# jeongminpark417/COALA-GNN

Hardware: AMD Instinct MI355X
Metric: feature-gather GB/s (payload = rows x dim x 4 B delivered per second), IGB-medium GraphSAGE minibatch fetch (higher is better)
Workload: dtype f32

## Files before the change

coala-gnn_amd/csrc/coala_cache.hip:

```cpp
#include <hip/hip_runtime.h>
#include <hip/hip_ext.h>

#include <algorithm>
#include <cstdarg>
#include <cstdio>
#include <cstdlib>
#include <cstring>
#include <new>
#include <type_traits>
#include <utility>
#include <vector>

#include "../../include/coala_hip.h"
#include "coala_internal.h"

namespace {

constexpr uint64_t kEmptyKey = 0xFFFFFFFFFFFFFFFFull;
constexpr uint32_t kLinkMiss = 0x80000000u;
constexpr uint32_t kLinkBad = 0x7FFFFFFFu;
constexpr int kStatBlocks = 2048;
constexpr int kFillSlots = 8;

struct CacheDev {
    void* keys;
    uint64_t* set_cnt;
    uint32_t* color_meta;
    int32_t* color_counters;
    const int32_t* node_color;
    float* lines;
    const float* cold;
    uint64_t num_sets;
    uint64_t num_rows;
    uint32_t cache_dim;
    uint32_t dim;
    uint32_t n_gpus;
    int32_t gshift;
    int32_t sshift;
    uint32_t distributed;
    uint32_t cold_partitioned;
    uint32_t tag32;
    uint64_t* set_head;
    uint32_t* miss_link;
    unsigned long long* stats;
};

__device__ __forceinline__ uint64_t set_of(const CacheDev& c, uint64_t id) {
    uint64_t k = id;
    if (c.distributed) {
        if (c.gshift >= 0) k = id >> c.gshift;
        else if ((id >> 32) == 0) k = (uint32_t)id / c.n_gpus;
        else k = id / c.n_gpus;
    }
    if (c.sshift >= 0) return k & (c.num_sets - 1);
    if ((k >> 32) == 0 && (c.num_sets >> 32) == 0) return (uint32_t)k % (uint32_t)c.num_sets;
    return k % c.num_sets;
}

__device__ __forceinline__ uint64_t cold_row_of(const CacheDev& c, uint64_t id) {
    if (!c.cold_partitioned) return id;
    if (c.gshift >= 0) return id >> c.gshift;
    return id / c.n_gpus;
}

constexpr int kMaxRanges = 64;
struct RangeSet {
    uint32_t n;
// ... 52 lines not shown
template <int CD, int VEC, int NP = 4>
struct Geo {
    static constexpr int UNITS = CD / VEC;
    static constexpr int LPR = UNITS >= 64 ? 64 : UNITS;
    static constexpr int RPP = 64 / LPR;
    static constexpr int VPL = UNITS / LPR;
    static constexpr int PASSES = (VPL >= 16) ? 1 : NP;
    static constexpr int R = RPP * PASSES;
};

constexpr int kK1MinWaves = 4;
constexpr int kK1Passes = 4;
constexpr int64_t kK1SingleMaxChunks = 1 << 20;
constexpr int kK1Waves = 2;
#ifdef COALA_DEV_KNOBS
constexpr int kK1MaxWaves = 4;
#else
constexpr int kK1MaxWaves = kK1Waves;
#endif

template <typename V> __device__ __forceinline__ V nt_load(const V* p) { return __builtin_nontemporal_load(p); }
template <typename V> __device__ __forceinline__ void nt_store(V v, V* p) { __builtin_nontemporal_store(v, p); }

template <int CD, int VEC, typename TAG, int NP, bool FULL, bool REDIR, bool SINGLE>
__global__ __launch_bounds__(64 * kK1MaxWaves, kK1MinWaves) void probe_gather_kernel(const int64_t* __restrict__ idx, float* __restrict__ out,
                                                                    int64_t n, uint32_t gen, uint32_t n_blocks, CacheDev c, Redirect rd) {
    using G = Geo<CD, VEC, NP>;
    using V = typename VecT<VEC>::type;
    using TG = TagGeo<TAG>;
    using TV = typename TG::vec;
    constexpr int R = G::R;
    static_assert(R <= 32, "per-chunk row masks are 32 bits wide");
    if (blockIdx.x == 0 && threadIdx.x < kFillSlots) reinterpret_cast<uint32_t*>(c.stats + 2 * kStatBlocks)[(gen & 1u) * kFillSlots + threadIdx.x] = 0u;
    uint32_t* fill_flag = reinterpret_cast<uint32_t*>(c.stats + 2 * kStatBlocks) + 2 * kFillSlots;
    if (blockIdx.x == 0 && threadIdx.x == kFillSlots) fill_flag[(gen + 1u) & 1u] = 0u;
    constexpr int TSTEPS = (R + TG::SPL - 1) / TG::SPL;
    int lane = threadIdx.x & 63;
#ifdef COALA_DEV_KNOBS
    const int wpb = (int)(blockDim.x >> 6);
#else
    constexpr int wpb = kK1Waves;
#endif
    const int64_t wave = (int64_t)blockIdx.x * wpb + (threadIdx.x >> 6);
    const int64_t n_waves = (int64_t)n_blocks * wpb;
    const int64_t n_chunks = (n + R - 1) / R;
    const uint32_t nunits = c.dim / VEC;
    const TAG* __restrict__ keys = reinterpret_cast<const TAG*>(c.keys);

    struct Ids { uint64_t id[TSTEPS]; bool valid[TSTEPS]; int32_t drow[REDIR ? TSTEPS : 1]; };
    struct Tags { uint64_t id[TSTEPS]; uint32_t set[TSTEPS]; TV kk[TSTEPS]; bool ok[TSTEPS]; bool valid[TSTEPS]; int32_t drow[REDIR ? TSTEPS : 1]; };
    auto load_ids = [&](int64_t chunk) {
        Ids r;
#pragma unroll
        for (int t = 0; t < TSTEPS; ++t) {
            const int q_l = t * TG::SPL + lane / TG::LPS;
// ... 15 lines not shown
            r.id[t] = ids.id[t];
            r.valid[t] = ids.valid[t];
            if (REDIR) r.drow[t] = ids.drow[t];
            r.ok[t] = ids.valid[t] && ids.id[t] < c.num_rows;
            r.set[t] = r.ok[t] ? (uint32_t)set_of(c, ids.id[t]) : 0u;
            r.kk[t] = TV(TG::EMPTY);
            if (r.ok[t]) r.kk[t] = *reinterpret_cast<const TV*>(keys + (uint64_t)r.set[t] * COALA_WAYS + (lane % TG::LPS) * TG::KPL);
        }
        return r;
    };

    int64_t chunk = wave;
    Ids ids_next = load_ids(chunk);
    Tags tags = load_tags(ids_next);
    if (!SINGLE) ids_next = load_ids(chunk + n_waves);

    for (; chunk < n_chunks; chunk += n_waves) {
        asm volatile("" : "+v"(lane));
        const int64_t base = chunk * R;
        uint32_t slot_v[TSTEPS];
        int32_t drow_v[REDIR ? TSTEPS : 1];
        uint64_t hit_b[TSTEPS], bad_b[TSTEPS];
        bool lead_l[TSTEPS], imiss_l[TSTEPS], bad_l[TSTEPS];
        unsigned long long prev[TSTEPS];
        const uint32_t lane_way0 = (uint32_t)((lane % TG::LPS) * TG::KPL);
#pragma unroll
        for (int t = 0; t < TSTEPS; ++t) {
            const TAG want = (TAG)tags.id[t];
            uint32_t way = 0xFFu;
#pragma unroll
            for (int k = TG::KPL - 1; k >= 0; --k)
                if (tags.kk[t][k] == want) way = lane_way0 + (uint32_t)k;
            if (!tags.ok[t]) way = 0xFFu;
            way = umin_u32(way, dpp_u32<0xB1>(way));
            way = umin_u32(way, dpp_u32<0x4E>(way));
            way = umin_u32(way, dpp_u32<0x141>(way));
            if (TG::LPS == 16) way = umin_u32(way, dpp_u32<0x140>(way));
            const bool hit = way != 0xFFu;
            slot_v[t] = tags.set[t] * COALA_WAYS + (way & (COALA_WAYS - 1));
            if (REDIR) drow_v[t] = tags.drow[t];
            hit_b[t] = __ballot(hit);
            bad_l[t] = tags.valid[t] && !tags.ok[t];
            bad_b[t] = __ballot(bad_l[t]);
            lead_l[t] = tags.valid[t] && (lane % TG::LPS) == 0;
            imiss_l[t] = lead_l[t] && tags.ok[t] && !hit;
            prev[t] = 0;
            if (imiss_l[t]) {
                const unsigned long long tag = ((unsigned long long)gen << 32) | (unsigned long long)(base + t * TG::SPL + lane / TG::LPS + 1);
                prev[t] = atomicExch(reinterpret_cast<unsigned long long*>(c.set_head + tags.set[t]), tag);
            }
        }
        {
            bool any = false;
#pragma unroll
            for (int t = 0; t < TSTEPS; ++t) any = any || imiss_l[t] || bad_l[t];
            if (__ballot(any) != 0 && lane == 0) fill_flag[gen & 1u] = 1u;
        }
        auto row_slot = [&](int q) { return (uint32_t)__builtin_amdgcn_readlane((int)slot_v[q / TG::SPL], TG::LPS * (q % TG::SPL)); };
        auto row_hit = [&](int q) { return ((hit_b[q / TG::SPL] >> (TG::LPS * (q % TG::SPL))) & 1) != 0; };
        auto row_bad = [&](int q) { return ((bad_b[q / TG::SPL] >> (TG::LPS * (q % TG::SPL))) & 1) != 0; };
        Ids ids_next2;
        if (!SINGLE) ids_next2 = load_ids(chunk + 2 * n_waves);

        const int sub = (G::RPP == 2) ? (lane >> 5) : 0;
        const int l_in = lane & (G::LPR - 1);
        V val[G::PASSES][G::VPL];
#pragma unroll
        for (int p = 0; p < G::PASSES; ++p) {
            const uint32_t s_a = row_slot(p * G::RPP), s_b = row_slot(p * G::RPP + (G::RPP - 1));
            const bool h_a = row_hit(p * G::RPP), h_b = row_hit(p * G::RPP + (G::RPP - 1));
            const uint32_t s = (G::RPP == 2 && sub) ? s_b : s_a;
            const bool h = (G::RPP == 2 && sub) ? h_b : h_a;
            const V* src = reinterpret_cast<const V*>(c.lines + (uint64_t)s * CD);
#pragma unroll
            for (int v = 0; v < G::VPL; ++v) {
                const uint32_t u = v * G::LPR + l_in;
                if (h && (FULL || u < nunits)) val[p][v] = nt_load(src + u);
            }
        }
        if (!SINGLE) {
            tags = load_tags(ids_next);
            ids_next = ids_next2;
        }
#pragma unroll
        for (int p = 0; p < G::PASSES; ++p) {
            const int q = p * G::RPP + sub;
            const bool h_a = row_hit(p * G::RPP), h_b = row_hit(p * G::RPP + (G::RPP - 1));
            const bool bad_a = row_bad(p * G::RPP), bad_b2 = row_bad(p * G::RPP + (G::RPP - 1));
            const bool h = (G::RPP == 2 && sub) ? h_b : h_a;
            const bool bad = (G::RPP == 2 && sub) ? bad_b2 : bad_a;
            V* dst = reinterpret_cast<V*>(out + (base + q) * (int64_t)c.dim);
            if (REDIR) {
                auto row_drow = [&](int r) { return (int32_t)__builtin_amdgcn_readlane(drow_v[r / TG::SPL], TG::LPS * (r % TG::SPL)); };
                const int32_t dr_a = row_drow(p * G::RPP), dr_b = row_drow(p * G::RPP + (G::RPP - 1));
                const int32_t dr = (G::RPP == 2 && sub) ? dr_b : dr_a;
                if (dr >= 0) dst = reinterpret_cast<V*>(rd.out + (int64_t)dr * (int64_t)c.dim);
            }
#pragma unroll
            for (int v = 0; v < G::VPL; ++v) {
                const uint32_t u = v * G::LPR + l_in;
                if (FULL || u < nunits) {
                    if (h) dst[u] = val[p][v];
                    else if (bad) dst[u] = V(0.0f);
                }
            }
        }
#pragma unroll
        for (int t = 0; t < TSTEPS; ++t) {
            if (lead_l[t]) {
                uint32_t w = 0u;
                if (imiss_l[t]) w = kLinkMiss | (((uint32_t)(prev[t] >> 32) == gen) ? (uint32_t)prev[t] : 0u);
                else if (bad_l[t]) w = kLinkBad;
                c.miss_link[base + t * TG::SPL + lane / TG::LPS] = w;
            }
        }
        if (SINGLE) break;
    }
}

__device__ __forceinline__ uint64_t shfl64(uint64_t v, int src) {
    const uint32_t lo = __shfl((int)(uint32_t)v, src), hi = __shfl((int)(uint32_t)(v >> 32), src);
    return ((uint64_t)hi << 32) | lo;
}

template <int CD, int VEC, bool REDIR = false, int NP = 4>
__global__ __launch_bounds__(256) void miss_fill_kernel(CacheDev c, const int64_t* __restrict__ idx, float* __restrict__ out,
                                                        int tile_rows, int sparse_max, uint32_t gen, RangeSet rs, Redirect rd, int dyn_slot) {
    using G = Geo<CD, VEC, NP>;
    using V = typename VecT<VEC>::type;
    constexpr int R = G::R;
    const int lane = threadIdx.x & 63;
    const int64_t wave = (int64_t)blockIdx.x * (blockDim.x >> 6) + (threadIdx.x >> 6);
    const int64_t n_waves = (int64_t)gridDim.x * (blockDim.x >> 6);
    const int64_t n_tiles = ((int64_t)rs.total + tile_rows - 1) / tile_rows;
    const int chunks_per_tile = tile_rows / R;
    const uint32_t nunits = c.dim / VEC;
    const int sub = (G::RPP == 2) ? (lane >> 5) : 0;
    const int l_in = lane & (G::LPR - 1);
    uint32_t my_miss = 0, my_bad = 0;

    constexpr int U = 8;
    uint32_t* ticket = reinterpret_cast<uint32_t*>(c.stats + 2 * kStatBlocks) + (dyn_slot < 0 ? 0 : dyn_slot);
    const bool dyn = dyn_slot >= 0;
    if (reinterpret_cast<const uint32_t*>(c.stats + 2 * kStatBlocks)[2 * kFillSlots + (gen & 1u)] == 0u) return;
    const int64_t n_deal = dyn ? 1 : n_waves;
    const int64_t even8 = n_tiles / (n_waves * 8);
    const int claim_min = even8 < 1 ? 1 : (even8 > U ? U : (int)even8);
    int claim = claim_min;
    for (int64_t unit = dyn ? -1 : wave;;) {
      int64_t claim_end = n_tiles;
      if (dyn) {
          uint32_t t = 0;
          if (lane == 0) t = atomicAdd(ticket, (uint32_t)claim);
          unit = (int64_t)(uint32_t)__builtin_amdgcn_readfirstlane((int)t);
          if (unit >= n_tiles) break;
          claim_end = unit + claim < n_tiles ? unit + claim : n_tiles;
          claim = claim * 2 > 4 * U ? 4 * U : claim * 2;
      } else if (unit >= n_tiles) break;
     for (int64_t tile0 = unit; tile0 < claim_end; tile0 += n_deal * U) {
      const int n_here = dyn ? (int)(claim_end - tile0 < U ? claim_end - tile0 : U) : U;
      uint64_t st_pack = 0;
#pragma unroll
      for (int u = 0; u < U; ++u) {
          const int64_t tile = tile0 + u * n_deal;
          const uint32_t p = (u < n_here && tile < n_tiles && lane < tile_rows) ? pos_of(rs, (uint32_t)(tile * tile_rows + lane)) : 0xFFFFFFFFu;
          const uint32_t w = (p != 0xFFFFFFFFu) ? c.miss_link[p] : 0u;
          const uint64_t v = (w == 0u) ? 0u : ((w & kLinkMiss) ? 1u : 2u);
          st_pack |= v << (8 * u);
      }
      if (!__ballot(st_pack != 0)) continue;
      uint32_t slot_l = 0, win_l = 0;
      uint64_t id_l = 0;
      int64_t drow_l = 0;
      auto rank_at = [&](uint32_t pos) {
          id_l = (uint64_t)idx[pos];
          drow_l = (int64_t)pos;
          if (REDIR && (int64_t)pos >= rd.begin && (int64_t)pos < rd.end)
              drow_l = -((rd.row_map ? rd.row_map[(int64_t)pos - rd.begin] : (int64_t)pos - rd.begin) + 1);
          const uint64_t set = set_of(c, id_l);
          uint32_t cur = (uint32_t)c.set_head[set];
          uint32_t total = 0, rank = 0;
          while (cur) {
              const uint32_t p2 = cur - 1;
              ++total;
              rank += (p2 < pos) ? 1u : 0u;
              cur = c.miss_link[p2] & ~kLinkMiss;
          }
          const uint64_t cv = __hip_atomic_load(c.set_cnt + set, __ATOMIC_RELAXED, __HIP_MEMORY_SCOPE_AGENT);
          const uint32_t cnt0 = ((uint32_t)(cv >> 32) == gen) ? (uint32_t)cv - total : (uint32_t)cv;
          if (rank == 0) __hip_atomic_store(c.set_cnt + set, ((uint64_t)gen << 32) | (uint32_t)(cnt0 + total), __ATOMIC_RELAXED, __HIP_MEMORY_SCOPE_AGENT);
          const uint32_t way = (cnt0 + rank) & (COALA_WAYS - 1);
          slot_l = (uint32_t)(set * COALA_WAYS) + way;
          win_l = (rank + COALA_WAYS >= total) ? 1u : 0u;
          if (win_l) {
              if (c.tag32) reinterpret_cast<uint32_t*>(c.keys)[slot_l] = (uint32_t)id_l;
              else reinterpret_cast<uint64_t*>(c.keys)[slot_l] = id_l;
              if (c.color_counters) {
                  const int32_t col = c.node_color[id_l];
                  atomicSub(c.color_counters + c.color_meta[slot_l], 1);
                  atomicAdd(c.color_counters + col, 1);
                  c.color_meta[slot_l] = (uint32_t)col;
              }
          }
      };
      auto move_group = [&](const int (&srcl)[G::PASSES], const bool (&live)[G::PASSES]) {
          V val[G::PASSES][G::VPL];
          uint32_t slot_[G::PASSES];
          uint64_t id[G::PASSES];
          int64_t drow[G::PASSES];
          bool winner[G::PASSES];
#pragma unroll
          for (int p = 0; p < G::PASSES; ++p) {
              slot_[p] = (uint32_t)__shfl((int)slot_l, srcl[p]);
              winner[p] = __shfl((int)win_l, srcl[p]) != 0;
              id[p] = shfl64(id_l, srcl[p]);
              drow[p] = (int64_t)shfl64((uint64_t)drow_l, srcl[p]);
          }
#pragma unroll
          for (int p = 0; p < G::PASSES; ++p) {
              const V* src = reinterpret_cast<const V*>(c.cold + cold_row_of(c, id[p]) * (uint64_t)c.dim);
#pragma unroll
              for (int v = 0; v < G::VPL; ++v) {
                  const uint32_t u = v * G::LPR + l_in;
                  if (live[p] && u < nunits) val[p][v] = nt_load(src + u);
              }
// ... 40 lines not shown
          const uint32_t cnt = (uint32_t)__builtin_popcountll(mmask[u]);
          total_miss += cnt;
          worst = cnt > worst ? cnt : worst;
      }
      if (!total_miss) continue;
      claim = claim_min;
      if (total_miss <= 64 && (int)worst <= sparse_max) {
          uint32_t k = (uint32_t)lane;
          int u_sel = -1;
          uint64_t m_sel = 0;
#pragma unroll
          for (int u = 0; u < U; ++u) {
              const uint32_t cnt = (uint32_t)__builtin_popcountll(mmask[u]);
              if (u_sel < 0) {
                  if (k < cnt) { u_sel = u; m_sel = mmask[u]; }
                  else k -= cnt;
              }
          }
          if (u_sel >= 0) {
              for (uint32_t i = 0; i < k; ++i) m_sel &= m_sel - 1;
              const uint32_t pos = pos_of(rs, (uint32_t)((tile0 + u_sel * n_deal) * tile_rows + __builtin_ctzll(m_sel)));
              rank_at(pos);
          }
          stream_holders(total_miss >= 64 ? ~0ull : ((1ull << total_miss) - 1ull));
          continue;
      }
#pragma nounroll
      for (int u = 0; u < U; ++u) {
        const uint8_t st = (uint8_t)(st_pack >> (8 * u));
        const uint64_t tile_mask = __ballot(st == 1);
        if (!tile_mask) continue;
        const uint32_t pos_l = st ? pos_of(rs, (uint32_t)((tile0 + u * n_deal) * tile_rows + lane)) : 0u;
        if (__builtin_popcountll(tile_mask) <= sparse_max) {
            if (st == 1) rank_at(pos_l);
            stream_holders(tile_mask);
        } else {
            int srcl[G::PASSES];
            bool live[G::PASSES];
            for (int ck = 0; ck < chunks_per_tile; ++ck) {
                const uint32_t live_mask = (uint32_t)(tile_mask >> (ck * R)) & ((1u << R) - 1u);
                if (!live_mask) continue;
                const int lane0 = ck * R;
                if (st == 1 && lane >= lane0 && lane < lane0 + R) rank_at(pos_l);
#pragma unroll
                for (int p = 0; p < G::PASSES; ++p) {
                    const int q = p * G::RPP + sub;
                    live[p] = (live_mask >> q) & 1;
                    srcl[p] = lane0 + q;
                }
                move_group(srcl, live);
            }
        }
      }
     }
      if (!dyn) break;
    }
    __shared__ uint32_t s_m[256 / 64], s_b[256 / 64];
    for (int off = 32; off > 0; off >>= 1) { my_miss += __shfl_down(my_miss, off); my_bad += __shfl_down(my_bad, off); }
    if (lane == 0) { s_m[threadIdx.x >> 6] = my_miss; s_b[threadIdx.x >> 6] = my_bad; }
    __syncthreads();
    if (threadIdx.x == 0) {
        uint32_t m = 0, b = 0;
        for (int w = 0; w < (int)(blockDim.x >> 6); ++w) { m += s_m[w]; b += s_b[w]; }
        if (m) c.stats[2 * blockIdx.x] += m;
        if (b) c.stats[2 * blockIdx.x + 1] += b;
    }
// ... 124 lines not shown
            if ((uint32_t)lane == g) off += __builtin_popcountll(mask);
        }
        if (valid) {
            node_out[dest] = id;
            map_out[dest] = i;
        }
    }
}

}


namespace {

struct LaunchShape {
    int k1_grid_cap;
    int k1_waves;
    bool k1_single;
    int k1_passes;
    int k2_grid_cap;
    int k2_tile_rows;
    int k2_sparse_max;
    int k2_unit_tiles;
};

LaunchShape launch_shape(uint32_t cache_dim, bool host_tier) {
    LaunchShape s;
    s.k1_grid_cap = 16384;
    s.k1_waves = kK1Waves;
    s.k1_single = cache_dim >= 256;
    s.k1_passes = 0;
    const int host_blocks = std::min(64, std::max(24, 16 * 1024 / (int)cache_dim));
    s.k2_grid_cap = host_tier ? host_blocks : kStatBlocks;
    s.k2_tile_rows = host_tier ? 64 : 0;
    s.k2_sparse_max = host_tier ? 32 : 0;
    s.k2_unit_tiles = host_tier ? 1 : 0;
    return s;
}

#ifdef COALA_DEV_KNOBS
void apply_dev_knobs(LaunchShape& s) {
    if (const char* e = getenv("COALA_K1_PASSES")) { int v = atoi(e); if (v == 2 || v == 4 || v == 8 || v == 16) s.k1_passes = v; }
    if (const char* e = getenv("COALA_K1_GRID")) { int g = atoi(e); if (g >= 1 && g <= 65535) s.k1_grid_cap = g; }
    if (const char* e = getenv("COALA_K1_WAVES")) { int w = atoi(e); if (w == 1 || w == 2 || w == 4) s.k1_waves = w; }
    if (const char* e = getenv("COALA_K1_SINGLE")) s.k1_single = atoi(e) != 0;
    if (const char* e = getenv("COALA_K2_TILE_ROWS")) { int t = atoi(e); if (t == 0 || t == 8 || t == 16 || t == 32 || t == 64) s.k2_tile_rows = t; }
    if (const char* e = getenv("COALA_K2_GRID")) { int g = atoi(e); if (g >= 1 && g <= kStatBlocks) s.k2_grid_cap = g; }
    if (const char* e = getenv("COALA_K2_SPARSE")) { int g = atoi(e); if (g >= 0 && g <= 64) s.k2_sparse_max = g; }
    if (const char* e = getenv("COALA_K2_UNIT_TILES")) { int g = atoi(e); if (g >= 0 && g <= 1) s.k2_unit_tiles = g; }
}
#endif

}

struct coala_cache {
    coala_cache_config_t cfg;
    CacheDev d;
    uint64_t cap = 0;
    uint32_t gen = 0;
    int32_t* node_color_dev = nullptr;
    uint32_t* wave_counts = nullptr;
    uint64_t wave_counts_cap = 0;
    int64_t* route_bases = nullptr;
    struct EvPair { hipEvent_t a, b; int kind; uint64_t rows; };
    std::vector<EvPair> ev_live;
    std::vector<hipEvent_t> ev_pool;
    coala_cache_profile_t prof{};
    hipStream_t last_stream = nullptr;
    hipStream_t order_stream = nullptr;
    bool order_set = false;
    hipEvent_t order_ev = nullptr;
    uint64_t table_bytes = 0;
    LaunchShape shape;
    int32_t* color_pin = nullptr;
    int32_t* color_pin_async = nullptr;
    hipEvent_t color_ev = nullptr;
    int32_t color_pending = -1;
    int64_t open_batch_rows = -1;
    std::vector<std::pair<int64_t, int64_t>> open_filled;
    int64_t open_filled_rows = 0;
    Redirect open_redirect{0, 0, nullptr, nullptr};
    int fill_launches = 0;
    uint64_t rows_total = 0;
    uint64_t cum_hit = 0, cum_miss = 0;
    uint64_t prof_hit0 = 0, prof_miss0 = 0;
    bool fetch_events = false;
    static constexpr int kFetchRing = 2048;
    std::vector<hipEvent_t> fev;
    uint64_t fev_calls = 0;
    hipEvent_t last_begin = nullptr, last_end = nullptr;
};

namespace {

#define fail coala_fail_
#define HIPCHK COALA_HIPCHK

int follow_stream(coala_cache* h, hipStream_t s) {
    if (h->order_set && h->order_stream != s) {
        if (!h->order_ev) HIPCHK(hipEventCreateWithFlags(&h->order_ev, hipEventDisableTiming));
        if (hipEventRecord(h->order_ev, h->order_stream) == hipSuccess) HIPCHK(hipStreamWaitEvent(s, h->order_ev, 0));
        else (void)hipGetLastError();
    }
    h->order_stream = s;
    h->order_set = true;
    return COALA_OK;
}

int ilog2_exact(uint64_t v) {
    if (v == 0 || (v & (v - 1))) return -1;
    int s = 0;
    while ((1ull << s) != v) ++s;
    return s;
}

int ensure_scratch(coala_cache* h, uint64_t n, hipStream_t s) {
    if (n <= h->cap) return COALA_OK;
    HIPCHK(hipStreamSynchronize(s));
    uint64_t cap = h->cap ? h->cap : 1024;
    while (cap < n) cap *= 2;
    if (h->d.miss_link) HIPCHK(hipFree(h->d.miss_link));
    h->d.miss_link = nullptr;
    HIPCHK(hipMalloc((void**)&h->d.miss_link, cap * sizeof(uint32_t)));
    h->cap = cap;
    return COALA_OK;
}

hipEvent_t take_event(coala_cache* h) {
    if (!h->ev_pool.empty()) {
        hipEvent_t e = h->ev_pool.back();
        h->ev_pool.pop_back();
        return e;
    }
    hipEvent_t e = nullptr;
    if (hipEventCreate(&e) != hipSuccess) return nullptr;
    return e;
}

void drain_events(coala_cache* h) {
    for (auto& p : h->ev_live) {
        float ms = 0.f;
        if (hipEventSynchronize(p.b) == hipSuccess && hipEventElapsedTime(&ms, p.a, p.b) == hipSuccess) {
            if (p.kind == 0) { h->prof.gather_ms += ms; h->prof.gather_launches++; h->prof.gather_rows += p.rows; }
            else { h->prof.fill_ms += ms; h->prof.fill_launches++; }
        }
        h->ev_pool.push_back(p.a);
        h->ev_pool.push_back(p.b);
    }
    h->ev_live.clear();
}

struct ProfScope {
    coala_cache* h; hipStream_t s; int kind; uint64_t rows; hipEvent_t a = nullptr, b = nullptr; bool on;
    hipEvent_t xa = nullptr, xb = nullptr;
    ProfScope(coala_cache* h_, hipStream_t s_, int kind_, uint64_t rows_, hipEvent_t xa_ = nullptr, hipEvent_t xb_ = nullptr)
        : h(h_), s(s_), kind(kind_), rows(rows_), xa(xa_), xb(xb_) {
        on = (h->cfg.flags & COALA_FLAG_PROFILE) != 0;
        if (on) {
            if (h->ev_live.size() >= 8192) drain_events(h);
            a = take_event(h); b = take_event(h);
            on = a && b;
            if (on) h->last_stream = s;
        }
    }
    template <typename K, typename... Args>
    void launch(K kernel, dim3 grid, dim3 block, Args... args) {
// ... 91 lines not shown
    d.num_rows = cfg->num_rows;
    d.cache_dim = (uint32_t)cd;
    d.dim = (uint32_t)cfg->dim;
    d.n_gpus = (uint32_t)cfg->n_gpus;
    d.gshift = ilog2_exact((uint64_t)cfg->n_gpus);
    d.sshift = ilog2_exact(sets);
    d.distributed = (cfg->flags & COALA_FLAG_DISTRIBUTED) ? 1u : 0u;
    d.cold_partitioned = (cfg->flags & COALA_FLAG_COLD_PARTITIONED) ? 1u : 0u;
    d.cold = cfg->cold_table;
    d.tag32 = (!(cfg->flags & COALA_FLAG_TAG64) && cfg->num_rows <= 0xFFFFFFFFull) ? 1u : 0u;
    const uint64_t tag_bytes = d.tag32 ? 4 : 8;
    int rc = COALA_OK;
    auto alloc = [&](void** p, uint64_t bytes) -> int {
        hipError_t e = hipMalloc(p, bytes);
        if (e != hipSuccess) return fail(COALA_ENOMEM, "hipMalloc(%llu) failed: %s", (unsigned long long)bytes, hipGetErrorString(e));
        h->table_bytes += bytes;
        return COALA_OK;
    };
    do {
        if ((rc = alloc((void**)&d.keys, slots * tag_bytes))) break;
        if ((rc = alloc((void**)&d.set_cnt, sets * 8))) break;
        if ((rc = alloc((void**)&d.color_meta, slots * 4))) break;
        if ((rc = alloc((void**)&d.set_head, sets * 8))) break;
        if ((rc = alloc((void**)&d.stats, (kStatBlocks * 2 + kFillSlots + 1) * 8))) break;
        if ((rc = alloc((void**)&d.lines, slots * (uint64_t)cd * 4))) break;
        if ((rc = alloc((void**)&h->route_bases, 65 * 8))) break;
        if (hipMemset(d.keys, 0xFF, slots * tag_bytes) != hipSuccess || hipMemset(d.set_cnt, 0, sets * 8) != hipSuccess ||
            hipMemset(d.color_meta, 0, slots * 4) != hipSuccess || hipMemset(d.set_head, 0, sets * 8) != hipSuccess ||
            hipMemset(d.stats, 0, (kStatBlocks * 2 + kFillSlots + 1) * 8) != hipSuccess) {
            rc = fail(COALA_EHIP, "hipMemset failed");
            break;
        }
        if (cfg->node_color) {
            if ((rc = alloc((void**)&d.color_counters, ((uint64_t)cfg->num_colors + 1) * 4))) break;
            if (hipMemset(d.color_counters, 0, ((uint64_t)cfg->num_colors + 1) * 4) != hipSuccess) { rc = fail(COALA_EHIP, "hipMemset failed"); break; }
            if ((rc = alloc((void**)&h->node_color_dev, cfg->num_rows * 4))) break;
            const uint64_t chunk = 1ull << 22;
            std::vector<int32_t> tmp((size_t)(cfg->num_rows < chunk ? cfg->num_rows : chunk));
            for (uint64_t off = 0; off < cfg->num_rows && rc == COALA_OK; off += chunk) {
                const uint64_t cnt = cfg->num_rows - off < chunk ? cfg->num_rows - off : chunk;
                for (uint64_t k = 0; k < cnt; ++k) {
                    const int64_t col = cfg->node_color[off + k];
                    if (col < 0 || col > cfg->num_colors) { rc = fail(COALA_EINVAL, "node_color[%llu]=%lld outside [0,%d]", (unsigned long long)(off + k), (long long)col, cfg->num_colors); break; }
                    tmp[k] = (int32_t)col;
                }
                if (rc == COALA_OK && hipMemcpy(h->node_color_dev + off, tmp.data(), cnt * 4, hipMemcpyHostToDevice) != hipSuccess)
                    rc = fail(COALA_EHIP, "colour upload failed");
            }
            if (rc) break;
            d.node_color = h->node_color_dev;
        }
// ... 7 lines not shown
            apply_dev_knobs(h->shape);
#endif
        }
        if (cfg->max_batch) rc = ensure_scratch(h, cfg->max_batch, nullptr);
    } while (0);
    if (rc == COALA_OK && hipDeviceSynchronize() != hipSuccess) rc = fail(COALA_EHIP, "device sync failed after create");
    if (rc != COALA_OK) {
        coala_cache_destroy(h);
        return rc;
    }
    *out = h;
    return COALA_OK;
}

int coala_cache_destroy(coala_cache_t* h) {
    if (!h) return COALA_OK;
    (void)hipSetDevice(h->cfg.device);
    (void)hipDeviceSynchronize();
    drain_events(h);
    for (auto e : h->ev_pool) (void)hipEventDestroy(e);
    for (auto e : h->fev)
        if (e) (void)hipEventDestroy(e);
    CacheDev& d = h->d;
    void* ptrs[] = {d.keys, d.set_cnt, d.color_meta, d.set_head, d.stats, d.lines, d.color_counters,
                    h->node_color_dev, d.miss_link,
                    h->wave_counts, h->route_bases};
    for (void* p : ptrs)
        if (p) (void)hipFree(p);
    if (h->color_pin) (void)hipHostFree(h->color_pin);
    if (h->color_pin_async) (void)hipHostFree(h->color_pin_async);
    if (h->color_ev) (void)hipEventDestroy(h->color_ev);
    if (h->order_ev) (void)hipEventDestroy(h->order_ev);
    delete h;
    return COALA_OK;
}

int64_t coala_cache_row_dim(const coala_cache_t* h) { return h ? (int64_t)h->d.dim : 0; }

int coala_cache_fetch_events(coala_cache_t* h, int enable) {
    if (!h) return fail(COALA_EINVAL, "null handle");
    h->fetch_events = enable != 0;
    if (!h->fetch_events) h->last_begin = h->last_end = nullptr;
    return COALA_OK;
}

int coala_cache_last_fetch_events(const coala_cache_t* h, void** begin_ev, void** end_ev) {
    if (!h) return fail(COALA_EINVAL, "null handle");
    if (begin_ev) *begin_ev = (void*)h->last_begin;
// ... 75 lines not shown
            if (ends[k] > begins[k]) add.emplace_back(begins[k], ends[k]);
        }
        if (phases == kPhaseFill) {
            std::vector<std::pair<int64_t, int64_t>> all = h->open_filled;
            all.insert(all.end(), add.begin(), add.end());
            std::sort(all.begin(), all.end());
            for (size_t k = 1; k < all.size(); ++k)
                if (all[k].first < all[k - 1].second)
                    return fail(COALA_EINVAL, "fill range [%lld, %lld) overlaps positions that were already filled in this batch", (long long)all[k].first, (long long)all[k].second);
            h->open_filled.swap(all);
        }
        for (auto& r : add) fill_rows += r.second - r.first;
        if (fill_rows == 0 && !(phases & kPhaseProbe)) return COALA_OK;
    }
    hipStream_t s = (hipStream_t)stream;
    HIPCHK(hipSetDevice(h->cfg.device));
    if (int rc_ = follow_stream(h, s)) return rc_;
    int rc = ensure_scratch(h, (uint64_t)n, s);
    if (rc) return rc;
    if (phases & kPhaseProbe) {
        h->fill_launches = 0;
        if (++h->gen == 0) {
            HIPCHK(hipMemsetAsync(h->d.set_head, 0, h->d.num_sets * 8, s));
            HIPCHK(hipMemset2DAsync(reinterpret_cast<char*>(h->d.set_cnt) + 4, 8, 0, 4, h->d.num_sets, s));
            h->gen = 1;
        }
        if (!(phases & kPhaseFill)) {
            h->open_batch_rows = n;
            h->open_filled.clear();
            h->open_filled_rows = 0;
            h->open_redirect = rd;
        }
    }
    const uint32_t gen = h->gen;
    const bool redir = rd.end > rd.begin;
    const bool vec4 = (h->d.dim % 4 == 0) && aligned16(out) && aligned16(h->d.cold) && (!redir || aligned16(rd.out));
    CacheDev d = h->d;
    if (force_dist) d.distributed = 1u;
    hipEvent_t fe_begin = nullptr, fe_end = nullptr;
    if (h->fetch_events && phases == kPhaseBoth && !(h->cfg.flags & COALA_FLAG_PROFILE)) {
        if (h->fev.empty()) h->fev.assign(2 * (size_t)coala_cache::kFetchRing, nullptr);
        const size_t slot = (size_t)(h->fev_calls % coala_cache::kFetchRing);
        for (size_t k = 2 * slot; k < 2 * slot + 2; ++k)
            if (!h->fev[k]) HIPCHK(hipEventCreate(&h->fev[k]));
        fe_begin = h->fev[2 * slot];
        fe_end = h->fev[2 * slot + 1];
    }
    const bool own_ring = fe_begin != nullptr;
    if (!own_ring && !(h->cfg.flags & COALA_FLAG_PROFILE)) {
        fe_begin = (phases & kPhaseProbe) ? ext_begin : nullptr;
        fe_end = (phases & kPhaseFill) ? ext_end : nullptr;
    }
    int n_sets = 0, set_no = 0;
    if ((phases & kPhaseFill) && fill_rows > 0) {
        int live = 0;
        for (int k = 0; k < n_ranges; ++k) live += ends[k] > begins[k];
        n_sets = (live + kMaxRanges - 1) / kMaxRanges;
    }
    rc = dispatch_geo(d.cache_dim, vec4, [&](auto geo) -> int {
        constexpr int CD = geo_cd(geo);
        constexpr int VEC = geo_vec(geo);
        using G = Geo<CD, VEC>;
        if (phases & kPhaseProbe) {
            ProfScope ps(h, s, 0, (uint64_t)n, fe_begin, nullptr);
            if (rode) rode[0] = ps.on ? ps.a : fe_begin;
            const bool full = (VEC == 4) && ((int)d.dim == CD);
            auto launch_k1 = [&](auto tag_c, auto np_c) {
                using TAG = decltype(tag_c);
                constexpr int NP = decltype(np_c)::value;
                constexpr int NPR = (Geo<CD, VEC, NP>::R > 8) ? NP / 2 : NP;
                using GK = Geo<CD, VEC, NP>;
                using GR = Geo<CD, VEC, NPR>;
                const int64_t chunks = redir ? (n + GR::R - 1) / GR::R : (n + GK::R - 1) / GK::R;
                const LaunchShape& ls = h->shape;
                const bool single = ls.k1_single && chunks <= kK1SingleMaxChunks;
                const dim3 grid(grid_for(chunks, ls.k1_waves, single ? (int)((kK1SingleMaxChunks + ls.k1_waves - 1) / ls.k1_waves) : ls.k1_grid_cap)), block(64 * ls.k1_waves);
                auto pick = [&](auto single_c) {
                    constexpr bool S = decltype(single_c)::value;
                    if (redir) return full ? probe_gather_kernel<CD, VEC, TAG, NPR, true, true, S> : probe_gather_kernel<CD, VEC, TAG, NPR, false, true, S>;
                    return full ? probe_gather_kernel<CD, VEC, TAG, NP, true, false, S> : probe_gather_kernel<CD, VEC, TAG, NP, false, false, S>;
                };
                ps.launch(single ? pick(std::true_type{}) : pick(std::false_type{}), grid, block, idx, out, n, gen, (uint32_t)grid.x, d, rd);
            };
#ifdef COALA_DEV_KNOBS
            if (h->shape.k1_passes) {
                auto by_np = [&](auto tag_c) {
                    switch (h->shape.k1_passes) {
                        case 2: launch_k1(tag_c, std::integral_constant<int, 2>{}); break;
                        case 8: launch_k1(tag_c, std::integral_constant<int, 8>{}); break;
                        case 16: launch_k1(tag_c, std::integral_constant<int, (Geo<CD, VEC, 16>::R <= 32 ? 16 : 8)>{}); break;
                        default: launch_k1(tag_c, std::integral_constant<int, 4>{}); break;
                    }
                };
                if (d.tag32) by_np(uint32_t{}); else by_np(uint64_t{});
            } else
#endif
            if (d.tag32) launch_k1(uint32_t{}, std::integral_constant<int, kK1Passes>{});
            else launch_k1(uint64_t{}, std::integral_constant<int, kK1Passes>{});
        }
        if ((phases & kPhaseFill) && fill_rows > 0) {
            const int tile_rows = h->shape.k2_tile_rows > 0 ? h->shape.k2_tile_rows : G::R;
            return for_each_range_set(begins, ends, n_ranges, [&](const RangeSet& rs) -> int {
                const bool last_set = ++set_no == n_sets;
                ProfScope ps(h, s, 2, 0, nullptr, last_set ? fe_end : nullptr);
                if (rode && last_set) rode[1] = ps.on ? ps.b : fe_end;
                const int64_t tiles = ((int64_t)rs.total + tile_rows - 1) / tile_rows;
                const dim3 grid(grid_for(tiles, 4, h->shape.k2_grid_cap));
                const int64_t waves = (int64_t)grid.x * 4;
                int dyn_slot = -1;
                if (h->shape.k2_unit_tiles > 0 && tiles > waves && tiles < 0x7FFFFFFF && h->fill_launches < kFillSlots)
                    dyn_slot = (int)((gen & 1u) * kFillSlots) + h->fill_launches;
                h->fill_launches++;
                if (redir) ps.launch(miss_fill_kernel<CD, VEC, true>, grid, dim3(256), d, idx, out, tile_rows, h->shape.k2_sparse_max, gen, rs, rd, dyn_slot);
                else ps.launch(miss_fill_kernel<CD, VEC, false>, grid, dim3(256), d, idx, out, tile_rows, h->shape.k2_sparse_max, gen, rs, rd, dyn_slot);
                return COALA_OK;
            });
        }
        return COALA_OK;
    });
    if (rc) return rc;
    if (own_ring) {
        h->last_begin = fe_begin;
        h->last_end = fe_end;
        h->fev_calls++;
    }
    if (phases & kPhaseProbe) h->rows_total += (uint64_t)n;
    if (phases == kPhaseFill) {
        h->open_filled_rows += fill_rows;
        if (h->open_filled_rows == h->open_batch_rows) {
            h->open_batch_rows = -1;
            h->open_filled.clear();
            h->open_filled_rows = 0;
        }
    }
    HIPCHK(hipGetLastError());
    if (h->cfg.flags & COALA_FLAG_SYNC) HIPCHK(hipStreamSynchronize(s));
    return COALA_OK;
// ... 203 lines not shown
    if (keys) {
        if (h->d.tag32) {
            uint32_t* narrow = reinterpret_cast<uint32_t*>(keys);
            HIPCHK(hipMemcpy(narrow, h->d.keys, slots * 4, hipMemcpyDeviceToHost));
            for (uint64_t k = slots; k-- > 0;) keys[k] = narrow[k] == 0xFFFFFFFFu ? kEmptyKey : (uint64_t)narrow[k];
        } else {
            HIPCHK(hipMemcpy(keys, h->d.keys, slots * 8, hipMemcpyDeviceToHost));
        }
    }
    if (set_cnt) HIPCHK(hipMemcpy2D(set_cnt, 4, h->d.set_cnt, 8, 4, h->d.num_sets, hipMemcpyDeviceToHost));
    if (color_meta) HIPCHK(hipMemcpy(color_meta, h->d.color_meta, slots * 4, hipMemcpyDeviceToHost));
    return COALA_OK;
}

int coala_cache_profile(coala_cache_t* h, coala_cache_profile_t* out, int reset) {
    if (!h || !out) return fail(COALA_EINVAL, "null argument");
    HIPCHK(hipSetDevice(h->cfg.device));
    drain_events(h);
    uint64_t v0, v1, v2;
    int rc = read_stats(h, nullptr, &v0, &v1, &v2, false);
    if (rc) return rc;
    const uint64_t th = h->cum_hit + v0, tm = h->cum_miss + v1;
    h->prof.gather_hits = th - h->prof_hit0;
    h->prof.fill_rows = tm - h->prof_miss0;
    if (h->cfg.flags & COALA_FLAG_PROFILE) {
        std::vector<float> gaps;
        for (int i = 0; i < 16; ++i) {
            hipEvent_t a = take_event(h), b = take_event(h);
            if (!a || !b) break;
            float ms = 0.f;
            if (hipEventRecord(a, h->last_stream) == hipSuccess && hipEventRecord(b, h->last_stream) == hipSuccess &&
                hipEventSynchronize(b) == hipSuccess && hipEventElapsedTime(&ms, a, b) == hipSuccess)
                gaps.push_back(ms);
            h->ev_pool.push_back(a);
            h->ev_pool.push_back(b);
        }
        if (!gaps.empty()) {
            std::sort(gaps.begin(), gaps.end());
            h->prof.event_overhead_us = gaps[gaps.size() / 2] * 1e3;
        }
    }
    *out = h->prof;
    if (reset) { h->prof = coala_cache_profile_t{}; h->prof_hit0 = th; h->prof_miss0 = tm; }
    return COALA_OK;
}

}
```

Measured before the change: 81.63.

## Defer cache-hit copies from probe kernel into fill kernel blocks for host-tier reads

For host-tier whole-batch fetches, the probe kernel no longer copies hit rows. It records each hit's slot in a per-set hit chain, and extra blocks in the miss-fill launch copy those rows concurrently with the host-memory miss streaming. Fill winners that evict a slot first copy the still-pending hit rows out of it before overwriting. The aim is to overlap on-device hit traffic with slow cold-tier reads and shorten the probe kernel. In exchange it adds per-row hit-record writes, chain walks and eviction checks, plus subtle ordering logic between concurrent hit copies and line overwrites.

```diff
diff --git a/coala-gnn_amd/csrc/coala_cache.hip b/coala-gnn_amd/csrc/coala_cache.hip
--- a/coala-gnn_amd/csrc/coala_cache.hip
+++ b/coala-gnn_amd/csrc/coala_cache.hip
@@ -20,6 +20,7 @@
 constexpr uint32_t kLinkMiss = 0x80000000u;
 constexpr uint32_t kLinkBad = 0x7FFFFFFFu;
 constexpr int kStatBlocks = 2048;
+constexpr int kK2HitBlocks = 1024;
 constexpr int kFillSlots = 8;
 
 struct CacheDev {
@@ -43,6 +44,8 @@
     uint64_t* set_head;
     uint32_t* miss_link;
     unsigned long long* stats;
+    uint64_t* hit_head;
+    uint64_t* hit_rec;
 };
 
 __device__ __forceinline__ uint64_t set_of(const CacheDev& c, uint64_t id) {
@@ -141,7 +144,7 @@
 template <typename V> __device__ __forceinline__ V nt_load(const V* p) { return __builtin_nontemporal_load(p); }
 template <typename V> __device__ __forceinline__ void nt_store(V v, V* p) { __builtin_nontemporal_store(v, p); }
 
-template <int CD, int VEC, typename TAG, int NP, bool FULL, bool REDIR, bool SINGLE>
+template <int CD, int VEC, typename TAG, int NP, bool FULL, bool REDIR, bool SINGLE, bool GATHER = true>
 __global__ __launch_bounds__(64 * kK1MaxWaves, kK1MinWaves) void probe_gather_kernel(const int64_t* __restrict__ idx, float* __restrict__ out,
                                                                     int64_t n, uint32_t gen, uint32_t n_blocks, CacheDev c, Redirect rd) {
     using G = Geo<CD, VEC, NP>;
@@ -150,6 +153,7 @@
     using TV = typename TG::vec;
     constexpr int R = G::R;
     static_assert(R <= 32, "per-chunk row masks are 32 bits wide");
+    static_assert(GATHER || !REDIR, "the probe-only form serves whole-batch reads, which never redirect");
     if (blockIdx.x == 0 && threadIdx.x < kFillSlots) reinterpret_cast<uint32_t*>(c.stats + 2 * kStatBlocks)[(gen & 1u) * kFillSlots + threadIdx.x] = 0u;
     uint32_t* fill_flag = reinterpret_cast<uint32_t*>(c.stats + 2 * kStatBlocks) + 2 * kFillSlots;
     if (blockIdx.x == 0 && threadIdx.x == kFillSlots) fill_flag[(gen + 1u) & 1u] = 0u;
@@ -211,6 +215,7 @@
         int32_t drow_v[REDIR ? TSTEPS : 1];
         uint64_t hit_b[TSTEPS], bad_b[TSTEPS];
         bool lead_l[TSTEPS], imiss_l[TSTEPS], bad_l[TSTEPS];
+        bool ihit_l[TSTEPS];
         unsigned long long prev[TSTEPS];
         const uint32_t lane_way0 = (uint32_t)((lane % TG::LPS) * TG::KPL);
 #pragma unroll
@@ -233,10 +238,11 @@
             bad_b[t] = __ballot(bad_l[t]);
             lead_l[t] = tags.valid[t] && (lane % TG::LPS) == 0;
             imiss_l[t] = lead_l[t] && tags.ok[t] && !hit;
+            ihit_l[t] = !GATHER && lead_l[t] && hit;
             prev[t] = 0;
-            if (imiss_l[t]) {
+            if (imiss_l[t] || ihit_l[t]) {
                 const unsigned long long tag = ((unsigned long long)gen << 32) | (unsigned long long)(base + t * TG::SPL + lane / TG::LPS + 1);
-                prev[t] = atomicExch(reinterpret_cast<unsigned long long*>(c.set_head + tags.set[t]), tag);
+                prev[t] = atomicExch(reinterpret_cast<unsigned long long*>((GATHER || !hit ? c.set_head : c.hit_head) + tags.set[t]), tag);
             }
         }
         {
@@ -264,7 +270,7 @@
 #pragma unroll
             for (int v = 0; v < G::VPL; ++v) {
                 const uint32_t u = v * G::LPR + l_in;
-                if (h && (FULL || u < nunits)) val[p][v] = nt_load(src + u);
+                if (GATHER && h && (FULL || u < nunits)) val[p][v] = nt_load(src + u);
             }
         }
         if (!SINGLE) {
@@ -289,7 +295,7 @@
             for (int v = 0; v < G::VPL; ++v) {
                 const uint32_t u = v * G::LPR + l_in;
                 if (FULL || u < nunits) {
-                    if (h) dst[u] = val[p][v];
+                    if (GATHER && h) dst[u] = val[p][v];
                     else if (bad) dst[u] = V(0.0f);
                 }
             }
@@ -301,6 +307,8 @@
                 if (imiss_l[t]) w = kLinkMiss | (((uint32_t)(prev[t] >> 32) == gen) ? (uint32_t)prev[t] : 0u);
                 else if (bad_l[t]) w = kLinkBad;
                 c.miss_link[base + t * TG::SPL + lane / TG::LPS] = w;
+                if (ihit_l[t])
+                    c.hit_rec[base + t * TG::SPL + lane / TG::LPS] = ((uint64_t)slot_v[t] << 32) | (((uint32_t)(prev[t] >> 32) == gen) ? (uint32_t)prev[t] : 0u);
             }
         }
         if (SINGLE) break;
@@ -312,21 +320,82 @@
     return ((uint64_t)hi << 32) | lo;
 }
 
-template <int CD, int VEC, bool REDIR = false, int NP = 4>
+template <int CD, int VEC, bool REDIR = false, int NP = 4, bool HITS = false>
 __global__ __launch_bounds__(256) void miss_fill_kernel(CacheDev c, const int64_t* __restrict__ idx, float* __restrict__ out,
-                                                        int tile_rows, int sparse_max, uint32_t gen, RangeSet rs, Redirect rd, int dyn_slot) {
+                                                        int tile_rows, int sparse_max, uint32_t gen, RangeSet rs, Redirect rd, int dyn_slot,
+                                                        int fill_blocks) {
     using G = Geo<CD, VEC, NP>;
     using V = typename VecT<VEC>::type;
     constexpr int R = G::R;
     const int lane = threadIdx.x & 63;
+    static_assert(!(HITS && REDIR), "the hits are copied by the fill only for whole-batch reads, which never redirect");
     const int64_t wave = (int64_t)blockIdx.x * (blockDim.x >> 6) + (threadIdx.x >> 6);
-    const int64_t n_waves = (int64_t)gridDim.x * (blockDim.x >> 6);
+    const int64_t n_waves = (int64_t)fill_blocks * (blockDim.x >> 6);
     const int64_t n_tiles = ((int64_t)rs.total + tile_rows - 1) / tile_rows;
     const int chunks_per_tile = tile_rows / R;
     const uint32_t nunits = c.dim / VEC;
     const int sub = (G::RPP == 2) ? (lane >> 5) : 0;
     const int l_in = lane & (G::LPR - 1);
     uint32_t my_miss = 0, my_bad = 0;
+
+    auto slot_evicted = [&](uint32_t slot) -> bool {
+        const uint32_t set = slot / COALA_WAYS;
+        const uint64_t head = c.set_head[set];
+        if ((uint32_t)(head >> 32) != gen) return false;
+        uint32_t cur = (uint32_t)head, total = 0;
+        while (cur) { ++total; cur = c.miss_link[cur - 1] & ~kLinkMiss; }
+        const uint64_t cv = __hip_atomic_load(c.set_cnt + set, __ATOMIC_RELAXED, __HIP_MEMORY_SCOPE_AGENT);
+        const uint32_t cnt0 = ((uint32_t)(cv >> 32) == gen) ? (uint32_t)cv - total : (uint32_t)cv;
+        return total >= COALA_WAYS || ((slot - cnt0) & (COALA_WAYS - 1)) < total;
+    };
+    if (HITS && (int)blockIdx.x >= fill_blocks) {
+        const int64_t hw = wave - n_waves, n_hw = (int64_t)(gridDim.x - fill_blocks) * (blockDim.x >> 6);
+        const int64_t n_steps = ((int64_t)rs.total + 63) / 64;
+        for (int64_t step = hw; step < n_steps; step += n_hw) {
+            const uint32_t pos = ((step * 64 + lane) < (int64_t)rs.total) ? pos_of(rs, (uint32_t)(step * 64 + lane)) : 0xFFFFFFFFu;
+            uint32_t slot = 0;
+            bool keep = false;
+            if (pos != 0xFFFFFFFFu && c.miss_link[pos] == 0u) {
+                slot = (uint32_t)(c.hit_rec[pos] >> 32);
+                keep = !slot_evicted(slot);
+            }
+            uint64_t m = __ballot(keep);
+            while (m) {
+                uint32_t s_[G::PASSES], p_[G::PASSES];
+                bool live[G::PASSES];
+#pragma unroll
+                for (int p = 0; p < G::PASSES; ++p) {
+                    int l0 = -1, l1 = -1;
+                    if (m) { l0 = __builtin_ctzll(m); m &= m - 1; }
+                    if (G::RPP == 2 && m) { l1 = __builtin_ctzll(m); m &= m - 1; }
+                    const int l = (G::RPP == 2 && sub) ? l1 : l0;
+                    live[p] = l >= 0;
+                    s_[p] = (uint32_t)__shfl((int)slot, l >= 0 ? l : 0);
+                    p_[p] = (uint32_t)__shfl((int)pos, l >= 0 ? l : 0);
+                }
+                V val[G::PASSES][G::VPL];
+#pragma unroll
+                for (int p = 0; p < G::PASSES; ++p) {
+                    const V* src = reinterpret_cast<const V*>(c.lines + (uint64_t)s_[p] * CD);
+#pragma unroll
+                    for (int v = 0; v < G::VPL; ++v) {
+                        const uint32_t u = v * G::LPR + l_in;
+                        if (live[p] && u < nunits) val[p][v] = nt_load(src + u);
+                    }
+                }
+#pragma unroll
+                for (int p = 0; p < G::PASSES; ++p) {
+                    V* dst = reinterpret_cast<V*>(out + (uint64_t)p_[p] * c.dim);
+#pragma unroll
+                    for (int v = 0; v < G::VPL; ++v) {
+                        const uint32_t u = v * G::LPR + l_in;
+                        if (live[p] && u < nunits) dst[u] = val[p][v];
+                    }
+                }
+            }
+        }
+        return;
+    }
 
     constexpr int U = 8;
     uint32_t* ticket = reinterpret_cast<uint32_t*>(c.stats + 2 * kStatBlocks) + (dyn_slot < 0 ? 0 : dyn_slot);
@@ -359,6 +428,7 @@
       }
       if (!__ballot(st_pack != 0)) continue;
       uint32_t slot_l = 0, win_l = 0;
+      uint32_t hcur_l = 0;
       uint64_t id_l = 0;
       int64_t drow_l = 0;
       auto rank_at = [&](uint32_t pos) {
@@ -381,6 +451,10 @@
           const uint32_t way = (cnt0 + rank) & (COALA_WAYS - 1);
           slot_l = (uint32_t)(set * COALA_WAYS) + way;
           win_l = (rank + COALA_WAYS >= total) ? 1u : 0u;
+          if (HITS && win_l) {
+              const uint64_t hh = c.hit_head[set];
+              hcur_l = ((uint32_t)(hh >> 32) == gen) ? (uint32_t)hh : 0u;
+          }
           if (win_l) {
               if (c.tag32) reinterpret_cast<uint32_t*>(c.keys)[slot_l] = (uint32_t)id_l;
               else reinterpret_cast<uint64_t*>(c.keys)[slot_l] = id_l;
@@ -390,6 +464,26 @@
                   atomicAdd(c.color_counters + col, 1);
                   c.color_meta[slot_l] = (uint32_t)col;
               }
+          }
+      };
+      auto evict_copies = [&]() {
+          if (!HITS) return;
+          auto seek = [&]() {
+              while (hcur_l) {
+                  const uint64_t r = c.hit_rec[hcur_l - 1];
+                  if ((uint32_t)(r >> 32) == slot_l) break;
+                  hcur_l = (uint32_t)r;
+              }
+          };
+          seek();
+          for (uint64_t m = __ballot(hcur_l != 0); m; m = __ballot(hcur_l != 0)) {
+              const int l = __builtin_ctzll(m);
+              const uint32_t p = (uint32_t)__builtin_amdgcn_readlane((int)hcur_l, l) - 1u;
+              const uint32_t s = (uint32_t)__builtin_amdgcn_readlane((int)slot_l, l);
+              const V* src = reinterpret_cast<const V*>(c.lines + (uint64_t)s * CD);
+              V* dst = reinterpret_cast<V*>(out + (uint64_t)p * c.dim);
+              for (uint32_t u = (uint32_t)lane; u < nunits; u += 64) dst[u] = src[u];
+              if (lane == l) { hcur_l = (uint32_t)c.hit_rec[p]; seek(); }
           }
       };
       auto move_group = [&](const int (&srcl)[G::PASSES], const bool (&live)[G::PASSES]) {
@@ -476,6 +570,7 @@
               const uint32_t pos = pos_of(rs, (uint32_t)((tile0 + u_sel * n_deal) * tile_rows + __builtin_ctzll(m_sel)));
               rank_at(pos);
           }
+          evict_copies();
           stream_holders(total_miss >= 64 ? ~0ull : ((1ull << total_miss) - 1ull));
           continue;
       }
@@ -487,6 +582,7 @@
         const uint32_t pos_l = st ? pos_of(rs, (uint32_t)((tile0 + u * n_deal) * tile_rows + lane)) : 0u;
         if (__builtin_popcountll(tile_mask) <= sparse_max) {
             if (st == 1) rank_at(pos_l);
+            evict_copies();
             stream_holders(tile_mask);
         } else {
             int srcl[G::PASSES];
@@ -496,6 +592,7 @@
                 if (!live_mask) continue;
                 const int lane0 = ck * R;
                 if (st == 1 && lane >= lane0 && lane < lane0 + R) rank_at(pos_l);
+                evict_copies();
 #pragma unroll
                 for (int p = 0; p < G::PASSES; ++p) {
                     const int q = p * G::RPP + sub;
@@ -666,6 +763,7 @@
     int k2_tile_rows;
     int k2_sparse_max;
     int k2_unit_tiles;
+    bool hit_in_fill;
 };
 
 LaunchShape launch_shape(uint32_t cache_dim, bool host_tier) {
@@ -679,6 +777,7 @@
     s.k2_tile_rows = host_tier ? 64 : 0;
     s.k2_sparse_max = host_tier ? 32 : 0;
     s.k2_unit_tiles = host_tier ? 1 : 0;
+    s.hit_in_fill = host_tier;
     return s;
 }
 
@@ -692,6 +791,7 @@
     if (const char* e = getenv("COALA_K2_GRID")) { int g = atoi(e); if (g >= 1 && g <= kStatBlocks) s.k2_grid_cap = g; }
     if (const char* e = getenv("COALA_K2_SPARSE")) { int g = atoi(e); if (g >= 0 && g <= 64) s.k2_sparse_max = g; }
     if (const char* e = getenv("COALA_K2_UNIT_TILES")) { int g = atoi(e); if (g >= 0 && g <= 1) s.k2_unit_tiles = g; }
+    if (const char* e = getenv("COALA_HIT_IN_FILL")) s.hit_in_fill = atoi(e) != 0;
 }
 #endif
 
@@ -728,6 +828,7 @@
     uint64_t rows_total = 0;
     uint64_t cum_hit = 0, cum_miss = 0;
     uint64_t prof_hit0 = 0, prof_miss0 = 0;
+    uint64_t prof_probe_only_rows = 0;
     bool fetch_events = false;
     static constexpr int kFetchRing = 2048;
     std::vector<hipEvent_t> fev;
@@ -766,6 +867,9 @@
     if (h->d.miss_link) HIPCHK(hipFree(h->d.miss_link));
     h->d.miss_link = nullptr;
     HIPCHK(hipMalloc((void**)&h->d.miss_link, cap * sizeof(uint32_t)));
+    if (h->d.hit_rec) HIPCHK(hipFree(h->d.hit_rec));
+    h->d.hit_rec = nullptr;
+    HIPCHK(hipMalloc((void**)&h->d.hit_rec, cap * sizeof(uint64_t)));
     h->cap = cap;
     return COALA_OK;
 }
@@ -785,7 +889,8 @@
     for (auto& p : h->ev_live) {
         float ms = 0.f;
         if (hipEventSynchronize(p.b) == hipSuccess && hipEventElapsedTime(&ms, p.a, p.b) == hipSuccess) {
-            if (p.kind == 0) { h->prof.gather_ms += ms; h->prof.gather_launches++; h->prof.gather_rows += p.rows; }
+            if (p.kind == 0 || p.kind == 3) { h->prof.gather_ms += ms; h->prof.gather_launches++; h->prof.gather_rows += p.rows; }
+            if (p.kind == 3) h->prof_probe_only_rows += p.rows;
             else { h->prof.fill_ms += ms; h->prof.fill_launches++; }
         }
         h->ev_pool.push_back(p.a);
@@ -923,11 +1028,13 @@
         if ((rc = alloc((void**)&d.set_cnt, sets * 8))) break;
         if ((rc = alloc((void**)&d.color_meta, slots * 4))) break;
         if ((rc = alloc((void**)&d.set_head, sets * 8))) break;
+        if ((rc = alloc((void**)&d.hit_head, sets * 8))) break;
         if ((rc = alloc((void**)&d.stats, (kStatBlocks * 2 + kFillSlots + 1) * 8))) break;
         if ((rc = alloc((void**)&d.lines, slots * (uint64_t)cd * 4))) break;
         if ((rc = alloc((void**)&h->route_bases, 65 * 8))) break;
         if (hipMemset(d.keys, 0xFF, slots * tag_bytes) != hipSuccess || hipMemset(d.set_cnt, 0, sets * 8) != hipSuccess ||
             hipMemset(d.color_meta, 0, slots * 4) != hipSuccess || hipMemset(d.set_head, 0, sets * 8) != hipSuccess ||
+            hipMemset(d.hit_head, 0, sets * 8) != hipSuccess ||
             hipMemset(d.stats, 0, (kStatBlocks * 2 + kFillSlots + 1) * 8) != hipSuccess) {
             rc = fail(COALA_EHIP, "hipMemset failed");
             break;
@@ -981,8 +1088,8 @@
     for (auto e : h->fev)
         if (e) (void)hipEventDestroy(e);
     CacheDev& d = h->d;
-    void* ptrs[] = {d.keys, d.set_cnt, d.color_meta, d.set_head, d.stats, d.lines, d.color_counters,
-                    h->node_color_dev, d.miss_link,
+    void* ptrs[] = {d.keys, d.set_cnt, d.color_meta, d.set_head, d.hit_head, d.stats, d.lines, d.color_counters,
+                    h->node_color_dev, d.miss_link, d.hit_rec,
                     h->wave_counts, h->route_bases};
     for (void* p : ptrs)
         if (p) (void)hipFree(p);
@@ -1104,6 +1211,7 @@
         h->fill_launches = 0;
         if (++h->gen == 0) {
             HIPCHK(hipMemsetAsync(h->d.set_head, 0, h->d.num_sets * 8, s));
+            HIPCHK(hipMemsetAsync(h->d.hit_head, 0, h->d.num_sets * 8, s));
             HIPCHK(hipMemset2DAsync(reinterpret_cast<char*>(h->d.set_cnt) + 4, 8, 0, 4, h->d.num_sets, s));
             h->gen = 1;
         }
@@ -1119,6 +1227,7 @@
     const bool vec4 = (h->d.dim % 4 == 0) && aligned16(out) && aligned16(h->d.cold) && (!redir || aligned16(rd.out));
     CacheDev d = h->d;
     if (force_dist) d.distributed = 1u;
+    const bool hit_in_fill = h->shape.hit_in_fill && phases == kPhaseBoth && !redir;
     hipEvent_t fe_begin = nullptr, fe_end = nullptr;
     if (h->fetch_events && phases == kPhaseBoth && !(h->cfg.flags & COALA_FLAG_PROFILE)) {
         if (h->fev.empty()) h->fev.assign(2 * (size_t)coala_cache::kFetchRing, nullptr);
@@ -1144,7 +1253,7 @@
         constexpr int VEC = geo_vec(geo);
         using G = Geo<CD, VEC>;
         if (phases & kPhaseProbe) {
-            ProfScope ps(h, s, 0, (uint64_t)n, fe_begin, nullptr);
+            ProfScope ps(h, s, hit_in_fill ? 3 : 0, (uint64_t)n, fe_begin, nullptr);
             if (rode) rode[0] = ps.on ? ps.a : fe_begin;
             const bool full = (VEC == 4) && ((int)d.dim == CD);
             auto launch_k1 = [&](auto tag_c, auto np_c) {
@@ -1159,6 +1268,7 @@
                 const dim3 grid(grid_for(chunks, ls.k1_waves, single ? (int)((kK1SingleMaxChunks + ls.k1_waves - 1) / ls.k1_waves) : ls.k1_grid_cap)), block(64 * ls.k1_waves);
                 auto pick = [&](auto single_c) {
                     constexpr bool S = decltype(single_c)::value;
+                    if (hit_in_fill) return full ? probe_gather_kernel<CD, VEC, TAG, NP, true, false, S, false> : probe_gather_kernel<CD, VEC, TAG, NP, false, false, S, false>;
                     if (redir) return full ? probe_gather_kernel<CD, VEC, TAG, NPR, true, true, S> : probe_gather_kernel<CD, VEC, TAG, NPR, false, true, S>;
                     return full ? probe_gather_kernel<CD, VEC, TAG, NP, true, false, S> : probe_gather_kernel<CD, VEC, TAG, NP, false, false, S>;
                 };
@@ -1187,14 +1297,17 @@
                 ProfScope ps(h, s, 2, 0, nullptr, last_set ? fe_end : nullptr);
                 if (rode && last_set) rode[1] = ps.on ? ps.b : fe_end;
                 const int64_t tiles = ((int64_t)rs.total + tile_rows - 1) / tile_rows;
-                const dim3 grid(grid_for(tiles, 4, h->shape.k2_grid_cap));
-                const int64_t waves = (int64_t)grid.x * 4;
+                const int fill_blocks = grid_for(tiles, 4, h->shape.k2_grid_cap);
+                const int hit_blocks = hit_in_fill ? grid_for(((int64_t)rs.total + 63) / 64, 4, kK2HitBlocks) : 0;
+                const dim3 grid(fill_blocks + hit_blocks);
+                const int64_t waves = (int64_t)fill_blocks * 4;
                 int dyn_slot = -1;
                 if (h->shape.k2_unit_tiles > 0 && tiles > waves && tiles < 0x7FFFFFFF && h->fill_launches < kFillSlots)
                     dyn_slot = (int)((gen & 1u) * kFillSlots) + h->fill_launches;
                 h->fill_launches++;
-                if (redir) ps.launch(miss_fill_kernel<CD, VEC, true>, grid, dim3(256), d, idx, out, tile_rows, h->shape.k2_sparse_max, gen, rs, rd, dyn_slot);
-                else ps.launch(miss_fill_kernel<CD, VEC, false>, grid, dim3(256), d, idx, out, tile_rows, h->shape.k2_sparse_max, gen, rs, rd, dyn_slot);
+                if (redir) ps.launch(miss_fill_kernel<CD, VEC, true>, grid, dim3(256), d, idx, out, tile_rows, h->shape.k2_sparse_max, gen, rs, rd, dyn_slot, fill_blocks);
+                else if (hit_in_fill) ps.launch(miss_fill_kernel<CD, VEC, false, 4, true>, grid, dim3(256), d, idx, out, tile_rows, h->shape.k2_sparse_max, gen, rs, rd, dyn_slot, fill_blocks);
+                else ps.launch(miss_fill_kernel<CD, VEC, false>, grid, dim3(256), d, idx, out, tile_rows, h->shape.k2_sparse_max, gen, rs, rd, dyn_slot, fill_blocks);
                 return COALA_OK;
             });
         }
@@ -1444,6 +1557,8 @@
     if (rc) return rc;
     const uint64_t th = h->cum_hit + v0, tm = h->cum_miss + v1;
     h->prof.gather_hits = th - h->prof_hit0;
+    if (h->prof_probe_only_rows && h->prof.gather_rows)
+        h->prof.gather_hits = (uint64_t)((double)h->prof.gather_hits * (double)(h->prof.gather_rows - h->prof_probe_only_rows) / (double)h->prof.gather_rows + 0.5);
     h->prof.fill_rows = tm - h->prof_miss0;
     if (h->cfg.flags & COALA_FLAG_PROFILE) {
         std::vector<float> gaps;
@@ -1463,8 +1578,8 @@
         }
     }
     *out = h->prof;
-    if (reset) { h->prof = coala_cache_profile_t{}; h->prof_hit0 = th; h->prof_miss0 = tm; }
-    return COALA_OK;
-}
-
-}
+    if (reset) { h->prof = coala_cache_profile_t{}; h->prof_hit0 = th; h->prof_miss0 = tm; h->prof_probe_only_rows = 0; }
+    return COALA_OK;
+}
+
+}
```

Result: no change. 82.20 (median of 6 runs) (+0.7%).
